# zichunhao/lgn-autoencoder

Hardware: AMD Instinct MI355X
Metric: jets/sec fwd+bwd, 30-particle maxdim=2 bs=512 (higher is better)
Workload: dtype f64

## Files before the change

### include/lgn_amd.h

```cpp
#ifndef LGN_AMD_H
#define LGN_AMD_H

#include <stddef.h>
#include <stdint.h>

#ifdef __cplusplus
extern "C" {
#endif

#define LGN_AMD_ABI_VERSION 19

int lgn_abi_version(void);
const char* lgn_last_error(void);

int lgn_level_fwd_f64(int B, int N, int C, int CO, int decoder,
                      const double* s_in, const double* v_in, const double* p, const uint8_t* mask,
                      const double* ra, const double* rb, const double* rc,
                      const double* w0, const double* b0, const double* w1, const double* b1,
                      const double* wm0, const double* wm1,
                      double* ag0, double* ag1, double* s_out, double* v_out, void* stream);

int lgn_level_bwd_partial_rows(int B, int N, int decoder, int* rows_mix, int* rows_rad);
int lgn_level_rad_partial_len(int C, int decoder);
int lgn_level_jet_split(int B, int N);
// ... 96 lines not shown
  double jet_loss_scale;
} lgn_net_desc;
#define LGN_REAL_SUM 0
#define LGN_REAL_REAL 1
#define LGN_REAL_IMAG 2
#define LGN_REAL_MEAN 3
#define LGN_REAL_NORM 4
#define LGN_LOSS_CHAMFER 0
#define LGN_LOSS_MSE 1
#define LGN_LOSS_HUNGARIAN 2
#define LGN_LOSS_EMD 3
typedef struct lgn_loss_desc {
  int kind;
  int abs_coord;
  int polar_coord;
  double scale;
} lgn_loss_desc;
#define LGN_POOL_MIN 0
#define LGN_POOL_MAX 1
#define LGN_POOL_MEAN 2
#define LGN_POOL_MIX 3
#define LGN_POOL(n, avg, o0, o1, o2, o3) ((n) | ((avg) << 3) | ((o0) << 4) | ((o1) << 6) | ((o2) << 8) | ((o3) << 10))
#define LGN_NET_NO_STATIC 1
#define LGN_NET_DEC_PAIRWISE 2
#define LGN_NET_LEVEL_V2 4
#define LGN_NET_MLP_V1 8
#define LGN_NET_MOMENTS_V1 16
#define LGN_NET_BWD_ORDERED 64
#define LGN_NET_DEC_UNFUSED 256
#define LGN_NET_MOMENTS_SPLIT 512
#define LGN_NET_MLP_BWD1 1024
#define LGN_NET_MLP_FULLTILE 2048
#define LGN_NET_LIVE_SCALARS 4096
#define LGN_NET_SPLIT_TAIL 128

#define LGN_LDS_LIMIT (160 * 1024)
long long lgn_encoder_end_lds_bytes(int N, int C0, int K, int CL, int Ts, int Tv, int pool);
long long lgn_decoder_end_lds_bytes(int N, int C0, int Tin, int CL);
long long lgn_junction_lds_bytes(int N, int CL, int Ts, int Tv, int pool, int C0);

int lgn_step_param_slots(const lgn_net_desc* d, int decoder);
long long lgn_step_workspace_doubles(const lgn_net_desc* d);
int lgn_step_fwd_bwd_f64(const lgn_net_desc* d, const double* params, double* grads, long long n_params,
                         const int64_t* enc_off, const int64_t* dec_off, const double* p4, const double* target,
                         const uint8_t* mask, const double* in_scalars, double* workspace, long long workspace_doubles,
                         double* recon, double* loss_part, const lgn_loss_desc* loss, int* assignment ,
                         int* status , void* stream);
#define LGN_FINALIZE_SCRATCH 2048
int lgn_step_finalize_f64(double* params, double* grads, long long n_params, const double* loss_part, int n_loss,
                          double l1_lambda, double* adam_m, double* adam_v, long long* step_dev,
                          double lr, double beta1, double beta2, double eps, int do_adam, double* loss_out, void* stream);
int lgn_step_train_f64(const lgn_net_desc* d, double* params, double* grads, long long n_params, const int64_t* enc_off,
                       const int64_t* dec_off, const double* p4, const double* target, const uint8_t* mask, const double* in_scalars,
                       double* workspace, long long workspace_doubles, double* recon, double* loss_part, int n_loss, double l1_lambda,
                       double* adam_m, double* adam_v, long long* step_dev, double lr, double beta1, double beta2, double eps,
                       int do_adam, double* loss_out, const lgn_loss_desc* loss, int* assignment ,
                       int* status , void* stream);

#define LGN_OPT_ADAM 0
#define LGN_OPT_RMSPROP 1
typedef struct {
  int kind;
  double l1_lambda, l2_lambda, lr, eps;
  double beta1, beta2;
  double alpha, momentum;
} lgn_optim_desc;
// ... 223 lines not shown
```

### lgn-autoencoder_amd/csrc/mlp_chain.hip

```cpp
#include "lds.hpp"
#include "ops.hpp"

namespace lgn {

namespace { LGN_STAMP_DECL }
#ifdef LGN_STAMPS
#define DSTAMP(i) do { if (threadIdx.x == 256 && blockIdx.x == 0) g_stamps[i] = clock64(); } while (0)
#else
#define DSTAMP(i) do { } while (0)
#endif
LGN_STAMP_READER(lgn_debug_stamps_mlp_chain)

namespace chain {

__host__ __device__ constexpr int stride2mod4(int x) { return x + ((6 - (x & 3)) & 3); }

__device__ __forceinline__ void lds_barrier() {
  __builtin_amdgcn_sched_barrier(0);
  __builtin_amdgcn_fence(__ATOMIC_RELEASE, "workgroup", "local");
  __builtin_amdgcn_s_barrier();
  __builtin_amdgcn_fence(__ATOMIC_ACQUIRE, "workgroup", "local");
  __builtin_amdgcn_sched_barrier(0);
}
template <int N, int P, class LoadF, class MmaF, class SideF>
// ... 223 lines not shown
  mfma_stream<N, LOOKAHEAD>(
      [&](int i) {
        const int u = It::tile(i), ks = It::ks(i);
        return u < NF ? wa[4 * ks * S + 16 * u] : wt[4 * ks * S + 4 * (u - NF)];
      },
      [&](int i, double av) {
        const int u = It::tile(i), ks = It::ks(i);
        if (u < NF) gin[u] = __builtin_amdgcn_mfma_f64_16x16x4f64(av, gpre[ks >> 2][ks & 3], gin[u], 0, 0, 0);
        else gin[NTO - 1][u - NF] = mfma4(av, gpre[ks >> 2][ks & 3], gin[NTO - 1][u - NF]);
      },
      [&](int i) {
        const int u = It::tile(i), ks = It::ks(i);
        constexpr int k1 = KS > 6 ? 5 : KS > 1 ? 1 : 0, k2 = KS > 6 ? 6 : KS > 2 ? 2 : k1, k3 = k2 + 1 < KS ? k2 + 1 : k2;
#pragma unroll
        for (int r = 0; r < 4; ++r)
          if (u > 0 && u < NF && ks == (r < 2 ? k1 : k2)) fin(u > 0 ? u - 1 : 0, r);
#pragma unroll
        for (int q = 0; q < NB; ++q)
          if (TH && u == 1 && NF > 1 && ks == k3) fin(NTO - 1, q);
        ext(i);
      });
}
template <class G, int NTO, bool TH_, class FinF>
__device__ __forceinline__ void fin_last(FinF fin, int r) {
  constexpr bool TH = TH_ && NTO == G::NT;
  if (!TH) fin(NTO - 1, r);
  else {
    fin(NTO - 2, r);
    if (NTO == 2 && r < G::NB) fin(NTO - 1, r);
  }
}

template <class G>
__device__ __forceinline__ double* saved_ptr(const MlpArgs<double>& a, int wave, int lane) {
  return a.h_saved + ((size_t)blockIdx.x * 4 + wave) * (G::NH * G::NT * 256) + lane * 4;
}
template <class G>
constexpr int saved_pieces() { return 2 * G::NT; }
template <class G, int NTI>
__device__ __forceinline__ void save_piece(double* hs, int l, const v4d (&h)[NTI], int j) {
  const v2d v = {h[j >> 1][2 * (j & 1)], h[j >> 1][2 * (j & 1) + 1]};
  __builtin_nontemporal_store(v, reinterpret_cast<v2d*>(hs + (l * G::NT + (j >> 1)) * 256 + 2 * (j & 1)));
}
template <class G>
__device__ __forceinline__ void load_piece(const double* hs, int l, v4d (&h)[G::NT], int j) {
  const v2d v = __builtin_nontemporal_load(reinterpret_cast<const v2d*>(hs + (l * G::NT + (j >> 1)) * 256 + 2 * (j & 1)));
  h[j >> 1][2 * (j & 1)] = v[0];
  h[j >> 1][2 * (j & 1) + 1] = v[1];
}

template <class G>
__device__ __forceinline__ void load_x(const MlpArgs<double>& a, int row, int g, v4d (&xb)[1]) {
  const bool rok = row < a.M;
#pragma unroll
  for (int r = 0; r < 4; ++r) {
    const int f = 4 * r + g;
    const bool ok = r < G::KS0 && rok && f < G::D;
    const double x = a.s_in[ok ? (size_t)(f & 1) * a.M * a.C + (size_t)row * a.C + (f >> 1) : 0];
    xb[0][r] = ok ? x : 0.0;
  }
}

template <int H, int D, bool GEN, bool SAVE, bool TWO = false, bool TH = false>
__global__ __launch_bounds__(TWO ? 512 : 256) void mlp_chain_fwd_kernel(MlpArgs<double> a) {
  using G = Geo<H, D>;
  const int tid = threadIdx.x, lane = tid & 63, wave = __builtin_amdgcn_readfirstlane(tid >> 6);
  const int c = lane & 15, g = lane >> 4;
  const int row = blockIdx.x * 64 + wave * 16 + c;
  extern __shared__ __align__(16) unsigned char smem_raw[];
  double* Wl = reinterpret_cast<double*>(smem_raw);
  WRegs<G> wrA, wrB;
  STAMP(0);
  STAMP_LIFE_BEGIN();
  if constexpr (TWO) {
    if (wave >= 4) {
      const int st = tid - 256;
      stage_prologue<G, false>(a, Wl, wrA, wrB, st);
      lds_barrier();
#define LGN_STAGE_STEP(Q)                                                                                            \
  _Pragma("unroll") for (int j = 0; j < stage_pieces<G>(); ++j) stage_piece<G, false, Q>(a, Wl, wrA, wrB, st, j);    \
  lds_barrier();
      LGN_STAGE_STEP(0) LGN_STAGE_STEP(1) LGN_STAGE_STEP(2) LGN_STAGE_STEP(3) LGN_STAGE_STEP(4) LGN_STAGE_STEP(5)
#undef LGN_STAGE_STEP
      return;
    }
  }
  v4d xb[1];
  load_x<G>(a, row, g, xb);
  if constexpr (!TWO) stage_prologue<G, false>(a, Wl, wrA, wrB, tid);
  lds_barrier();
  STAMP(1);
  v4d h0[G::NT], h1[G::NT];
  double* hs = SAVE ? saved_ptr<G>(a, wave, lane) : nullptr;
#define LGN_CHAIN_STEP(Q, HIN, HOUT, KS, NTI)                                                                        \
  layer_fwd<G, KS, NTI, GEN, TH, (Q == 3)>(Wl + (Q & 1) * G::WSIZE, HIN, HOUT, c, g, a.act, [&](int i) {           \
    constexpr int NI = Items<G, KS, TH>::N;                                                                          \
    if (!TWO && !LGN_DBG_NOSTAGE) deal<NI, stage_pieces<G>()>(i, [&](int j) { stage_piece<G, false, Q>(a, Wl, wrA, wrB, tid, j); });      \
    if (SAVE && Q > 0) deal<NI, 2 * NTI>(i, [&](int j) { save_piece<G>(hs, Q - 1, HIN, j); });                      \
  });                                                                                                                \
  lds_barrier();                                                                                                     \
  STAMP(2 + Q);
  LGN_CHAIN_STEP(0, xb, h0, G::KS0, 1)
  LGN_CHAIN_STEP(1, h0, h1, G::KSH, G::NT)
  LGN_CHAIN_STEP(2, h1, h0, G::KSH, G::NT)
  LGN_CHAIN_STEP(3, h0, h1, G::KSH, G::NT)
  LGN_CHAIN_STEP(4, h1, h0, G::KSH, G::NT)
  LGN_CHAIN_STEP(5, h0, h1, G::KSH, G::NT)
#undef LGN_CHAIN_STEP
  if (SAVE) {
#pragma unroll
    for (int j = 0; j < saved_pieces<G>(); ++j) save_piece<G>(hs, G::NH - 1, h1, j);
  }
  const v4d y = layer_out<G>(Wl + (G::NH & 1) * G::WSIZE, h1, c, g);
#pragma unroll
  for (int r = 0; r < 4; ++r) {
    const int o = 4 * r + g;
    if (o < D && row < a.M) a.s_out[mlp_out_index(a, o & 1, row, o >> 1)] = y[r];
  }
  STAMP(8);
  STAMP_LIFE_END();
}

template <class G, int NTI>
__device__ __forceinline__ void publish_piece(double* T, const v4d (&v)[NTI], int wave, int c, int g, int j) {
  T[(4 * j + g) * G::SR + 16 * wave + c] = v[j >> 2][j & 3];
}
template <class G, int L, int NU, class SideF>
__device__ __forceinline__ void dw_unit(const double* Gt, const double* Xt, double* part, int t, int u0, int c, int g, SideF side) {
  constexpr int SR = G::SR, HO = G::hout(L), HI = G::hin(L), N = 16 * NU, P = 6;
  const double* ga = Gt + (16 * t + c) * SR + g;
  const double* xb = Xt + (16 * u0 + c) * SR + g;
  double* pW = part + G::off_w(L);
  v4d acc[NU];
#pragma unroll
  for (int u = 0; u < NU; ++u) acc[u] = v4d{0, 0, 0, 0};
  double dbs = 0.0, qa[16], qx[N];
  auto load = [&](int i) {
    qx[i] = xb[16 * (i >> 4) * SR + 4 * (i & 15)];
    if (i < 16) qa[i] = ga[4 * i];
  };
  auto store = [&](int u, int r) {
    const int o = 16 * t + 4 * r + g, k = 16 * (u0 + u) + c;
    if (o < HO && k < HI) __builtin_nontemporal_store(acc[u][r], &pW[o * HI + k]);
  };
// ... 29 lines not shown
    if (wave < G::NT) { dw_unit<G, L, 1>(Gt, Xt, part, wave, 0, c, g, side); return true; }
  } else {
    const int t = (wave + L) & 3;
    if (t < G::NT) { dw_unit<G, L, G::NT>(Gt, Xt, part, t, 0, c, g, side); return true; }
  }
  return false;
}

template <int H, int D, bool GEN, bool SAVE, bool TH = false>
__global__ __launch_bounds__(256) void mlp_chain_bwd_kernel(MlpArgs<double> a) {
  using G = Geo<H, D>;
  constexpr int NT = G::NT, NH = G::NH;
  const int tid = threadIdx.x, lane = tid & 63, wave = __builtin_amdgcn_readfirstlane(tid >> 6);
  const int c = lane & 15, g = lane >> 4;
  const int row = blockIdx.x * 64 + wave * 16 + c;
  extern __shared__ __align__(16) unsigned char smem_raw[];
  double* Wl = reinterpret_cast<double*>(smem_raw);
  double* Gt = Wl + 2 * G::WSIZE;
  double* Xt = Gt + 2 * G::TSIZE;
  double* part = a.part + (size_t)blockIdx.x * a.psize;
  WRegs<G> wrA, wrB;
  STAMP(10);
  v4d xb[1];
  load_x<G>(a, row, g, xb);
  v4d gout[1];
#pragma unroll
  for (int r = 0; r < 4; ++r) {
    const int o = 4 * r + g;
    const bool ok = o < D && row < a.M;
    const double x = a.g_out[ok ? mlp_out_index(a, o & 1, row, o >> 1) : 0];
    gout[0][r] = ok ? x : 0.0;
  }
  v4d h[NH][NT];
  const double* hs = SAVE ? saved_ptr<G>(a, wave, lane) : nullptr;
  if constexpr (SAVE) {
    issue_image<G, NH>(a, wrA, tid);
    issue_image<G, NH - 1>(a, wrB, tid);
#pragma unroll
    for (int j = 0; j < saved_pieces<G>(); ++j) load_piece<G>(hs, NH - 1, h[NH - 1], j);
#pragma unroll
    for (int j = 0; j < saved_pieces<G>(); ++j) load_piece<G>(hs, NH - 2, h[NH - 2], j);
    commit_image<G, NH>(Wl, wrA, tid);
    issue_image<G, NH - 2>(a, wrA, tid);
    lds_barrier();
    STAMP(11);
  } else {
    stage_prologue<G, true>(a, Wl, wrA, wrB, tid);
    lds_barrier();
    STAMP(11);
#define LGN_CHAIN_STEP(Q, HIN, KS, NTI)                                                                              \
  layer_fwd<G, KS, NTI, GEN, TH>(Wl + (Q & 1) * G::WSIZE, HIN, h[Q], c, g, a.act, [&](int i) {                      \
    deal<Items<G, KS, TH>::N, stage_pieces<G>()>(i, [&](int j) { stage_piece<G, true, Q>(a, Wl, wrA, wrB, tid, j); });  \
  });                                                                                                                \
  lds_barrier();                                                                                                     \
  STAMP(12 + Q);
    LGN_CHAIN_STEP(0, xb, G::KS0, 1)
    LGN_CHAIN_STEP(1, h[0], G::KSH, NT)
    LGN_CHAIN_STEP(2, h[1], G::KSH, NT)
    LGN_CHAIN_STEP(3, h[2], G::KSH, NT)
    LGN_CHAIN_STEP(4, h[3], G::KSH, NT)
    LGN_CHAIN_STEP(5, h[4], G::KSH, NT)
#undef LGN_CHAIN_STEP
  }
  v4d gpA[NT] = {}, gpB[NT] = {}, gin[NT];
  {
    constexpr int NI = Items<G, G::KS0, TH>::N, NSV = SAVE && NH >= 3 ? saved_pieces<G>() : 0, NPC = 4 + 4 * NT + stage_pieces<G>() + NSV;
    auto fin = [&](int u, int r) {
      double y = gin[u][r] * act_slope_t<GEN>(h[NH - 1][u][r], a.act);
      pin(y);
      gpA[u][r] = y;
    };
    layer_bwd<G, G::KS0, NT, 1, TH>(Wl + 0 * G::WSIZE, gout, gin, c, g, fin, [&](int i) {
      deal<NI, NPC>(i, [&](int j) {
        if (j < 4) publish_piece<G, 1>(Gt, gout, wave, c, g, j);
        else if (j < 4 + 4 * NT) publish_piece<G, NT>(Xt, h[NH - 1], wave, c, g, j - 4);
        else if (j < 4 + 4 * NT + stage_pieces<G>()) stage_piece<G, true, NH>(a, Wl, wrA, wrB, tid, j - 4 - 4 * NT);
        else if constexpr (NSV > 0) load_piece<G>(hs, NH - 3, h[NH >= 3 ? NH - 3 : 0], j - 4 - 4 * NT - stage_pieces<G>());
      });
    });
#pragma unroll
    for (int r = 0; r < 4; ++r) fin_last<G, NT, TH>(fin, r);
    lds_barrier();
    STAMP(18);
  }
#define LGN_CHAIN_BSTEP(L, GP, GN)                                                                                   \
  {                                                                                                                  \
    constexpr int q_ = 2 * NH - (L), NI = Items<G, G::KSH, TH>::N, NSV = SAVE && (L) >= 3 ? saved_pieces<G>() : 0,               \
                  NPC = 8 * NT + stage_pieces<G>() + NSV;                                                            \
    auto fin = [&](int u, int r) {                                                                                   \
      double y = gin[u][r] * act_slope_t<GEN>(h[(L) - 1][u][r], a.act);                                              \
      pin(y);                                                                                                        \
      GN[u][r] = y;                                                                                                  \
    };                                                                                                               \
    layer_bwd<G, G::KSH, NT, NT, TH>(Wl + (q_ & 1) * G::WSIZE, GP, gin, c, g, fin, [&](int i) {                          \
      deal<NI, NPC>(i, [&](int j) {                                                                                  \
        if (j < 4 * NT) publish_piece<G, NT>(Gt + ((L) & 1) * G::TSIZE, GP, wave, c, g, j);                          \
        else if (j < 8 * NT) publish_piece<G, NT>(Xt + ((L) & 1) * G::TSIZE, h[(L) - 1], wave, c, g, j - 4 * NT);    \
        else if (j < 8 * NT + stage_pieces<G>()) stage_piece<G, true, q_>(a, Wl, wrA, wrB, tid, j - 8 * NT);         \
        else if constexpr (NSV > 0) load_piece<G>(hs, (L) - 3, h[(L) >= 3 ? (L) - 3 : 0], j - 8 * NT - stage_pieces<G>()); \
      });                                                                                                            \
    });                                                                                                              \
    auto tail = [&](int i) {                                                                                         \
      if (i == 1) { fin_last<G, NT, TH>(fin, 0); fin_last<G, NT, TH>(fin, 1); }                                                                \
      if (i == 2) { fin_last<G, NT, TH>(fin, 2); fin_last<G, NT, TH>(fin, 3); }                                                                \
    };                                                                                                               \
    if (!dw_layer<G, (L) + 1>(Gt + (((L) + 1) & 1) * G::TSIZE, Xt + (((L) + 1) & 1) * G::TSIZE, part, wave, c, g, tail)) {   \
      tail(1);                                                                                                       \
      tail(2);                                                                                                       \
    }                                                                                                                \
    lds_barrier();                                                                                                   \
    STAMP(12 + q_);                                                                                                  \
  }
  LGN_CHAIN_BSTEP(5, gpA, gpB)
  LGN_CHAIN_BSTEP(4, gpB, gpA)
  LGN_CHAIN_BSTEP(3, gpA, gpB)
  LGN_CHAIN_BSTEP(2, gpB, gpA)
  LGN_CHAIN_BSTEP(1, gpA, gpB)
#undef LGN_CHAIN_BSTEP
  {
    v4d gx[1];
    layer_bwd<G, G::KSH, 1, NT, TH>(Wl + 0 * G::WSIZE, gpB, gx, c, g, [&](int, int) {}, [&](int i) {
      deal<G::KSH, 4 * NT + 4>(i, [&](int j) {
        if (j < 4 * NT) publish_piece<G, NT>(Gt, gpB, wave, c, g, j);
        else publish_piece<G, 1>(Xt, xb, wave, c, g, j - 4 * NT);
      });
    });
    auto tail = [&](int i) {
      if (i >= 1 && i <= 4) {
        const int f = 4 * (i - 1) + g;
        if (f < D && row < a.M) a.g_in[mlp_out_index(a, f & 1, row, f >> 1)] = gx[0][i - 1];
      }
    };
// ... 91 lines not shown
#pragma unroll
  for (int i = 0; i < P; ++i) load(i);
  __builtin_amdgcn_sched_barrier(0);
#pragma unroll
  for (int i = 0; i < N; ++i) {
    if (i + P < N) load(i + P);
    if (i < 16) acc = __builtin_amdgcn_mfma_f64_16x16x4f64(qa[i], qx[i], acc, 0, 0, 0);
    else strip = mfma4(qa[i], qx[i], strip);
    if (i >= 17 && i <= 20) __builtin_nontemporal_store(acc[i - 17], &pW[(16 * t + 4 * (i - 17) + g) * H + 16 * u + c]);
    side(i);
    __builtin_amdgcn_sched_barrier(0);
  }
  __builtin_nontemporal_store(strip, tr ? &pW[(16 * u + c) * H + 32 + g] : &pW[(32 + g) * H + 16 * u + c]);
  if (w == 3) {
    const double* ca = Gt + (32 + (c & 3)) * SR + 16 * (c >> 2) + g;
    const double* cb = Xt + (32 + (c & 3)) * SR + 16 * (c >> 2) + g;
    double v = 0.0;
#pragma unroll
    for (int sk = 0; sk < 4; ++sk) v = mfma4(ca[4 * sk], cb[4 * sk], v);
    v += shfl_xor(v, 4);
    v += shfl_xor(v, 8);
    if (c < 4) __builtin_nontemporal_store(v, &pW[(32 + g) * H + 32 + c]);
  } else {
    double d4[4] = {0.0, 0.0, 0.0, 0.0};
#pragma unroll
    for (int sk = 0; sk < 16; ++sk) d4[sk & 3] += w == 1 ? qa[16 + sk] : qa[sk];
    double dbs = (d4[0] + d4[1]) + (d4[2] + d4[3]);
    dbs += shfl_xor(dbs, 16);
    dbs += shfl_xor(dbs, 32);
    if (g == 0 && (w != 1 || c < 4)) __builtin_nontemporal_store(dbs, &part[G::off_b(L) + (w == 1 ? 32 : 16 * t) + c]);
  }
}

template <int H, int D, bool GEN, bool TH = false>
__global__ __launch_bounds__(512) void mlp_chain_bwd2_kernel(MlpArgs<double> a) {
  using G = Geo<H, D>;
  constexpr int NT = G::NT, NH = G::NH;
  const int lane = threadIdx.x & 63, wave = __builtin_amdgcn_readfirstlane((int)threadIdx.x >> 6);
  const int w4 = wave & 3;
  const int c = lane & 15, g = lane >> 4;
  extern __shared__ __align__(16) unsigned char smem_raw[];
  double* Wl = reinterpret_cast<double*>(smem_raw);
  double* Gt = Wl + 2 * G::WSIZE;
  double* Xt = Gt + 2 * G::TSIZE;
  STAMP(10);
  if (wave >= 4) {
    __builtin_amdgcn_s_setprio(2);
    const int tid = (int)threadIdx.x - 256;
    double* part = a.part + (size_t)blockIdx.x * a.psize;
    WRegs<G> wrA, wrB;
    stage_prologue<G, true>(a, Wl, wrA, wrB, tid);
    lds_barrier();
#define LGN_STAGE_ALL(Q)                                                                                             \
  _Pragma("unroll") for (int j = 0; j < stage_pieces<G>(); ++j) stage_piece<G, true, Q>(a, Wl, wrA, wrB, tid, j);
#define LGN_STAGE_STEP(Q) LGN_STAGE_ALL(Q) lds_barrier();
    LGN_STAGE_STEP(0) LGN_STAGE_STEP(1) LGN_STAGE_STEP(2) LGN_STAGE_STEP(3) LGN_STAGE_STEP(4) LGN_STAGE_STEP(5)
    LGN_STAGE_STEP(6)
    constexpr bool THIN3 = TH && NT == 3 && G::R == 4, EVEN = NT == 3 && !THIN3;
    double* qs = Xt + 2 * G::TSIZE;
#define LGN_DW_STEP(L)                                                                                               \
  {                                                                                                                  \
    constexpr int q_ = 2 * NH - (L), NS = stage_pieces<G>(), L1 = (L) + 1;                                           \
    constexpr bool HID = EVEN && L1 >= 1 && L1 < NH, HID3 = THIN3 && L1 >= 1 && L1 < NH;                             \
    constexpr int NI = HID ? 36 : HID3 ? 32 : (L1 == NH || L1 == 0) ? 16 : 16 * NT;                                  \
    auto side = [&](int i) { deal<NI, NS>(i, [&](int j) { stage_piece<G, true, q_>(a, Wl, wrA, wrB, tid, j); }); };  \
    if constexpr (EVEN && L1 + 1 >= 1 && L1 + 1 < NH) {                                                              \
      if (w4 == 1) dw_quarter_sum<G, (L1 + 1 < NH ? L1 + 1 : 1)>(qs + ((L1 + 1) & 1) * 1024, part, lane, c, g);     \
    }                                                                                                                \
    if constexpr (HID3) {                                                                                            \
      dw_thin3<G, (HID3 ? L1 : 1)>(Gt + (L1 & 1) * G::TSIZE, Xt + (L1 & 1) * G::TSIZE, part, w4, c, g, side);        \
    } else if constexpr (HID) {                                                                                      \
      dw_hidden3<G, (HID ? L1 : 1)>(Gt + (L1 & 1) * G::TSIZE, Xt + (L1 & 1) * G::TSIZE, part, qs + (L1 & 1) * 1024, w4, lane, c, g, side); \
    } else if (!dw_layer<G, L1>(Gt + (L1 & 1) * G::TSIZE, Xt + (L1 & 1) * G::TSIZE, part, w4, c, g, side)) {         \
      LGN_STAGE_ALL(q_)                                                                                              \
    }                                                                                                                \
    DSTAMP(44 + (L));                                                                                                \
    lds_barrier();                                                                                                   \
  }
    LGN_DW_STEP(5) LGN_DW_STEP(4) LGN_DW_STEP(3) LGN_DW_STEP(2) LGN_DW_STEP(1) LGN_DW_STEP(0)
#undef LGN_DW_STEP
#undef LGN_STAGE_STEP
#undef LGN_STAGE_ALL
    if constexpr (EVEN && NH >= 2) {
      if (w4 == 1) dw_quarter_sum<G, 1>(qs + 1024, part, lane, c, g);
    }
    dw_layer<G, 0>(Gt, Xt, part, w4, c, g, [&](int) {});
    return;
  }
  const int row = blockIdx.x * 64 + wave * 16 + c;
  v4d xb[1];
  load_x<G>(a, row, g, xb);
  v4d gout[1];
#pragma unroll
  for (int r = 0; r < 4; ++r) {
    const int o = 4 * r + g;
    const bool ok = o < D && row < a.M;
    const double x = a.g_out[ok ? mlp_out_index(a, o & 1, row, o >> 1) : 0];
    gout[0][r] = ok ? x : 0.0;
  }
  v4d h[NH][NT];
  lds_barrier();
  STAMP(11);
#define LGN_CHAIN_STEP(Q, HIN, KS, NTI)                                                                              \
  layer_fwd<G, KS, NTI, GEN, TH>(Wl + (Q & 1) * G::WSIZE, HIN, h[Q], c, g, a.act, [&](int) {});                          \
  lds_barrier();                                                                                                     \
  STAMP(12 + Q);
  LGN_CHAIN_STEP(0, xb, G::KS0, 1)
  LGN_CHAIN_STEP(1, h[0], G::KSH, NT)
  LGN_CHAIN_STEP(2, h[1], G::KSH, NT)
  LGN_CHAIN_STEP(3, h[2], G::KSH, NT)
  LGN_CHAIN_STEP(4, h[3], G::KSH, NT)
  LGN_CHAIN_STEP(5, h[4], G::KSH, NT)
#undef LGN_CHAIN_STEP
  v4d gpA[NT] = {}, gpB[NT] = {}, gin[NT];
  {
    constexpr int NI = Items<G, G::KS0, TH>::N, NPC = 4 + 4 * NT;
    auto fin = [&](int u, int r) {
      double y = gin[u][r] * act_slope_t<GEN>(h[NH - 1][u][r], a.act);
      pin(y);
      gpA[u][r] = y;
    };
    layer_bwd<G, G::KS0, NT, 1, TH>(Wl + 0 * G::WSIZE, gout, gin, c, g, fin, [&](int i) {
      deal<NI, NPC>(i, [&](int j) {
        if (j < 4) publish_piece<G, 1>(Gt, gout, wave, c, g, j);
        else publish_piece<G, NT>(Xt, h[NH - 1], wave, c, g, j - 4);
      });
    });
#pragma unroll
    for (int r = 0; r < 4; ++r) fin_last<G, NT, TH>(fin, r);
    lds_barrier();
    STAMP(18);
  }
#define LGN_CHAIN_BSTEP(L, GP, GN)                                                                                   \
  {                                                                                                                  \
    constexpr int q_ = 2 * NH - (L), NI = Items<G, G::KSH, TH>::N, NPC = 8 * NT;                                                 \
    auto fin = [&](int u, int r) {                                                                                   \
      double y = gin[u][r] * act_slope_t<GEN>(h[(L) - 1][u][r], a.act);                                              \
      pin(y);                                                                                                        \
      GN[u][r] = y;                                                                                                  \
    };                                                                                                               \
    layer_bwd<G, G::KSH, NT, NT, TH>(Wl + (q_ & 1) * G::WSIZE, GP, gin, c, g, fin, [&](int i) {                          \
      deal<NI, NPC>(i, [&](int j) {                                                                                  \
        if (j < 4 * NT) publish_piece<G, NT>(Gt + ((L) & 1) * G::TSIZE, GP, wave, c, g, j);                          \
        else publish_piece<G, NT>(Xt + ((L) & 1) * G::TSIZE, h[(L) - 1], wave, c, g, j - 4 * NT);                    \
      });                                                                                                            \
    });                                                                                                              \
    STAMP(56 + (L));                                                                                                 \
    _Pragma("unroll") for (int r = 0; r < 4; ++r) fin_last<G, NT, TH>(fin, r);                                                    \
    STAMP(50 + (L));                                                                                                 \
    lds_barrier();                                                                                                   \
    STAMP(12 + q_);                                                                                                  \
  }
  LGN_CHAIN_BSTEP(5, gpA, gpB)
  LGN_CHAIN_BSTEP(4, gpB, gpA)
  LGN_CHAIN_BSTEP(3, gpA, gpB)
  LGN_CHAIN_BSTEP(2, gpB, gpA)
  LGN_CHAIN_BSTEP(1, gpA, gpB)
#undef LGN_CHAIN_BSTEP
  {
    v4d gx[1];
    layer_bwd<G, G::KSH, 1, NT, TH>(Wl + 0 * G::WSIZE, gpB, gx, c, g, [&](int, int) {}, [&](int i) {
      deal<G::KSH, 4 * NT + 4>(i, [&](int j) {
        if (j < 4 * NT) publish_piece<G, NT>(Gt, gpB, wave, c, g, j);
        else publish_piece<G, 1>(Xt, xb, wave, c, g, j - 4 * NT);
      });
    });
#pragma unroll
    for (int r = 0; r < 4; ++r) {
      const int f = 4 * r + g;
      if (f < D && row < a.M) a.g_in[mlp_out_index(a, f & 1, row, f >> 1)] = gx[0][r];
    }
    lds_barrier();
    STAMP(25);
  }
}

template <class G>
__device__ __forceinline__ double* saved_ptr16(const MlpArgs<double>& a, int lane) {
  return a.h_saved + (size_t)blockIdx.x * (G::NH * G::NT * 256) + lane * 4;
}
// ... 515 lines not shown
  using G = Geo<H, D, 128>;
  const int nblk = cdiv(a.M, 16);
  const size_t smem = backward ? G::bwd_bytes() : G::fwd_bytes();
  if (backward) LGN_CHECK_ARG(a.psize == G::psize(), "cgmlp: psize %d, expected %d", a.psize, G::psize());
  LGN_CHECK_ARG(!a.h_saved || a.h_rows >= nblk * 16, "cgmlp: the saved-activation buffer has %d rows per layer, %d rows need %d",
                a.h_rows, a.M, nblk * 16);
  void (*kern)(MlpArgs<double>);
  if (backward) kern = a.h_saved ? (a.act == 0 ? mlp_chain_bwd16_kernel<H, D, false, true> : mlp_chain_bwd16_kernel<H, D, true, true>)
                                 : (a.act == 0 ? mlp_chain_bwd16_kernel<H, D, false, false> : mlp_chain_bwd16_kernel<H, D, true, false>);
  else kern = a.h_saved ? (a.act == 0 ? mlp_chain_fwd16_kernel<H, D, false, true> : mlp_chain_fwd16_kernel<H, D, true, true>)
                        : (a.act == 0 ? mlp_chain_fwd16_kernel<H, D, false, false> : mlp_chain_fwd16_kernel<H, D, true, false>);
  return lds_launch(kern, "cgmlp (16-row)", dim3(nblk), dim3(backward ? 256 : 192), smem, stream, a);
}

template <int H, int D, bool TH>
static int launch_fwd(const MlpArgs<double>& a, hipStream_t stream) {
  using G = Geo<H, D>;
  static_assert(G::fwd_bytes() <= LGN_LDS_LIMIT, "LDS budget");
  const bool two = !(a.flags & LVL_MLP_BWD1);
  auto kern = two ? (a.act == 0 ? mlp_chain_fwd_kernel<H, D, false, false, true, TH> : mlp_chain_fwd_kernel<H, D, true, false, true, TH>)
                  : (a.act == 0 ? mlp_chain_fwd_kernel<H, D, false, false, false, TH> : mlp_chain_fwd_kernel<H, D, true, false, false, TH>);
  return lds_launch(kern, "cgmlp forward (wide)", dim3(cdiv(a.M, 64)), dim3(two ? 512 : 256), G::fwd_bytes(), stream, a);
}

template <int H, int D, bool TH>
static int launch(const MlpArgs<double>& a, bool backward, hipStream_t stream) {
  using G = Geo<H, D>;
  const int nblk = cdiv(a.M, 64);
  const size_t smem = backward ? G::bwd_bytes() : G::fwd_bytes();
  static_assert(G::bwd_bytes() <= LGN_LDS_LIMIT, "LDS budget");
  if (backward) LGN_CHECK_ARG(a.psize == G::psize(), "cgmlp: psize %d, expected %d", a.psize, G::psize());
  LGN_CHECK_ARG(!a.h_saved || a.h_rows >= nblk * 64, "cgmlp: the saved-activation buffer has %d rows per layer, %d rows need %d",
                a.h_rows, a.M, nblk * 64);
  if (backward && !a.h_saved && !(a.flags & LVL_MLP_BWD1)) {
    auto k2 = a.act == 0 ? mlp_chain_bwd2_kernel<H, D, false, TH> : mlp_chain_bwd2_kernel<H, D, true, TH>;
    const size_t smem2 = smem - (TH && G::NT == 3 && G::R == 4 ? sizeof(double) * 2 * 1024 : 0);
    return lds_launch(k2, "cgmlp backward (two roles)", dim3(nblk), dim3(512), smem2, stream, a);
  }
  if (!backward && !a.h_saved && !(a.flags & LVL_MLP_BWD1)) {
    auto k2 = a.act == 0 ? mlp_chain_fwd_kernel<H, D, false, false, true, TH> : mlp_chain_fwd_kernel<H, D, true, false, true, TH>;
    return lds_launch(k2, "cgmlp forward (two roles)", dim3(nblk), dim3(512), smem, stream, a);
  }
  auto kern = a.h_saved ? (a.act == 0 ? (backward ? mlp_chain_bwd_kernel<H, D, false, true, TH> : mlp_chain_fwd_kernel<H, D, false, true, false, TH>)
                                      : (backward ? mlp_chain_bwd_kernel<H, D, true, true, TH> : mlp_chain_fwd_kernel<H, D, true, true, false, TH>))
                        : (a.act == 0 ? (backward ? mlp_chain_bwd_kernel<H, D, false, false, TH> : mlp_chain_fwd_kernel<H, D, false, false, false, TH>)
                                      : (backward ? mlp_chain_bwd_kernel<H, D, true, false, TH> : mlp_chain_fwd_kernel<H, D, true, false, false, TH>));
  return lds_launch(kern, "cgmlp", dim3(nblk), dim3(256), smem, stream, a);
}
template <int H, int D>
static int launch_thin(const MlpArgs<double>& a, bool backward, hipStream_t stream) {
  static_assert(Geo<H, D>::THIN, "a last tile of at most eight neurons");
  return (a.flags & LVL_MLP_FULLTILE) ? launch<H, D, false>(a, backward, stream) : launch<H, D, true>(a, backward, stream);
}

}

int mlp_chain_dispatch(const MlpArgs<double>& a, bool backward, hipStream_t stream) {
  if ((a.flags & LVL_MLP_V1) || a.nlin != 7) return -2;
  if (mlp_rows_per_workgroup(a.M, a.H) != 64) {
    if (!(a.flags & LVL_MLP_BWD1) && (!backward || a.h_saved)) {
      if (a.H == 48 && a.C == 4) return chain::launch16s<48, 8>(a, backward, stream);
      if (a.H == 36 && a.C == 3) return chain::launch16s<36, 6>(a, backward, stream);
    }
    if (a.H == 48 && a.C == 4) return chain::launch16<48, 8>(a, backward, stream);
    if (a.H == 36 && a.C == 3) return chain::launch16<36, 6>(a, backward, stream);
    if (a.H == 24 && a.C == 2) return chain::launch16<24, 4>(a, backward, stream);
    if (a.H == 12 && a.C == 1) return chain::launch16<12, 2>(a, backward, stream);
    return -2;
  }
  if (a.H == 48 && a.C == 4) return chain::launch<48, 8, false>(a, backward, stream);
  if (a.H == 36 && a.C == 3) return chain::launch_thin<36, 6>(a, backward, stream);
  if (a.H == 24 && a.C == 2) return chain::launch_thin<24, 4>(a, backward, stream);
  if (a.H == 12 && a.C == 1) return chain::launch<12, 2, false>(a, backward, stream);
// ... 11 lines not shown
```

### lgn-autoencoder_amd/csrc/step.hip

```cpp
#include <stdlib.h>

#include <algorithm>
#include <vector>

#include "net.hpp"
#include "../../include/lgn_amd.h"

namespace lgn {
namespace {

inline size_t r16(size_t n) { return (n + 15) & ~size_t(15); }

struct Bump {
  double* base;
  size_t off = 0;
  double* here() const { return base ? base + off : nullptr; }
  double* take(size_t n) {
    double* p = here();
    off += r16(n);
    return p;
  }
};

struct Deferred {
// ... 228 lines not shown
}

bool stage_keeps_chamfer(const StageLoss* al) { return !al || (al->kind == LGN_LOSS_EMD && al->emd.chamfer_weight > 0.0); }
double chamfer_scale(const StageLoss* al) { return al ? al->emd.chamfer_weight : 1.0; }

int stage_loss_train(const StageLoss& L, int B, int N, int C, const double* v, const double* wo1, const double* target, int method,
                     double* recon, double* loss_part, double* g_v, double* part, hipStream_t st) {
  if (L.kind == LGN_LOSS_EMD) return dec_output_emd_loss(B, N, C, v, wo1, target, method, L.emd, recon, loss_part, g_v, part, st);
  return dec_output_assign_loss(B, N, C, v, wo1, target, method, L.al, recon, loss_part, g_v, part, st);
}
int stage_loss_eval(const StageLoss& L, int B, int N, int C, const double* v, const double* wo1, const double* target, int method,
                    double* recon_real, double* loss_part, hipStream_t st) {
  if (L.kind == LGN_LOSS_EMD) return dec_output_emd_eval(B, N, C, v, wo1, target, method, L.emd, recon_real, loss_part, st);
  return dec_output_assign_eval(B, N, C, v, wo1, target, method, L.al, recon_real, loss_part, st);
}

struct NetBuf {
  double *s[5], *v[5], *smix[4], *ag0[4], *ag1[4];
  double* hsave[4];
  double* sep[4];
};
void carve_net(Bump& b, const lgn_net_desc& d, bool dec, size_t BN, bool last_mlp_bwd, NetBuf& n) {
  const int* ch = dec ? d.dec_channels : d.enc_channels;
  const int L = d.n_levels;
  for (int l = 0; l <= L; ++l) {
    n.s[l] = b.take(2 * BN * ch[l]);
    n.v[l] = b.take(8 * BN * ch[l]);
  }
  for (int l = 0; l < L; ++l) {
    n.smix[l] = b.take(2 * BN * ch[l + 1]);
    n.ag0[l] = b.take(4 * BN * ch[l]);
    n.ag1[l] = b.take(16 * BN * ch[l]);
    n.sep[l] = dec ? b.take((size_t)d.B * sep_sums_doubles(ch[l])) : nullptr;
    const size_t hs = (last_mlp_bwd || l + 1 < L) && BN <= mlp_save_max_rows()
                          ? mlp_saved_doubles((int)BN, d.mlp_hidden_mul * 2 * ch[l + 1], d.mlp_nlin) : 0;
    n.hsave[l] = hs ? b.take(hs) : nullptr;
  }
}

struct BwdScratch {
  double *gs[2], *gv[2];
  double *gsmix, *g_ag;
  double *zeros_s, *g_p, *g_lat_s, *tail_cnt;
  size_t zero_doubles;
  double* zero0() const { return tail_cnt < zeros_s ? tail_cnt : zeros_s; }
  double* tot[4];
  double* parts;
  size_t parts_size;
};
void carve_level_grads(Bump& b, size_t BN, int cmax, BwdScratch& k) {
  for (int q = 0; q < 2; ++q) {
    k.gs[q] = b.take(2 * BN * cmax);
    k.gv[q] = b.take(8 * BN * cmax);
  }
  k.gsmix = b.take(2 * BN * cmax);
  k.g_ag = b.take(20 * BN * cmax);
}
inline size_t tot_doubles(int C, bool dec) { return rad_partial_size(C, dec) + 16; }

size_t net_parts(const lgn_net_desc& d, bool dec, int N) {
  const int* ch = dec ? d.dec_channels : d.enc_channels;
  int rm, rr;
  level_bwd_partial_rows(d.B, N, dec, d.flags, &rm, &rr);
  size_t sum = 0;
  for (int l = 0; l < d.n_levels; ++l) {
    const int H = d.mlp_hidden_mul * 2 * ch[l + 1];
    sum += r16((size_t)rm * 4 * ch[l + 1] * 5 * ch[l]) + r16((size_t)rr * rad_partial_size(ch[l], dec)) +
// ... 1153 lines not shown
```

### lgn-autoencoder_amd/lgn/_native.py

```python
from __future__ import annotations

import ctypes as C
import os
from typing import Optional, Sequence

import torch

_HERE = os.path.dirname(os.path.abspath(__file__))
LIB_PATH = os.environ.get("LGN_AMD_LIB") or os.path.join(_HERE, "_lib", "liblgn_amd.so")
ABI_VERSION = 19
FINALIZE_SCRATCH = 2048
FINALIZE_OPT_SCRATCH = 4096

_lib: Optional[C.CDLL] = None

_vp, _i, _ip = C.c_void_p, C.c_int, C.POINTER(C.c_int)

_SIGNATURES = {
    "lgn_level_fwd_f64": [_i] * 5 + [_vp] * 18,
    "lgn_level_bwd_partial_rows": [_i, _i, _i, _ip, _ip],
    "lgn_level_rad_partial_len": [_i, _i],
    "lgn_level_jet_split": [_i, _i],
    "lgn_cg_product_fwd_f64": [_i] * 8 + [_vp] * 7,
    "lgn_cg_product_bwd_f64": [_i] * 8 + [_vp] * 9,
# ... 54 lines not shown
            need = max(need, L.lgn_junction_lds_bytes(n, ch[-1], ts, tv, code, decoder.num_channels[0]))
    if decoder is not None:
        ch = decoder.num_channels
        need = max(need, L.lgn_decoder_end_lds_bytes(decoder.num_output_particles, ch[0], decoder.tau_latent_vectors, ch[-1]))
    return 0 <= need <= LDS_LIMIT


def pool_blocks(code: int) -> int:
    if code == 0:
        return 2
    return 1 if (code >> 3) & 1 else code & 7


class NetDesc(C.Structure):
    _fields_ = [("B", C.c_int), ("N", C.c_int), ("n_levels", C.c_int), ("enc_channels", C.c_int * 5),
                ("dec_channels", C.c_int * 5), ("tau_s", C.c_int), ("tau_v", C.c_int), ("mlp_hidden_mul", C.c_int),
                ("mlp_nlin", C.c_int), ("tau_v_in", C.c_int),
                ("enc_tables", _tp * 4), ("dec_tables", _tp * 4),
                ("enc_Q", C.c_int * 5), ("enc_qs", C.c_int * 5), ("enc_qv", C.c_int * 5),
                ("dec_Q", C.c_int * 5), ("dec_qs", C.c_int * 5), ("dec_qv", C.c_int * 5), ("flags", C.c_int),
                ("activation", C.c_int), ("n_in_scalars", C.c_int), ("latent_pool", C.c_int), ("dec_N", C.c_int),
                ("get_real", C.c_int), ("jet_loss_scale", C.c_double)]

    def __init__(self, *a, **kw):
        super().__init__(*a, **kw)
        self.flags = net_flags()


NET_NO_STATIC = 1
_NET_FLAG_ENV = {"LGN_AMD_NO_STATIC": 1, "LGN_AMD_DEC_PAIRWISE": 2, "LGN_AMD_LEVEL_V2": 4, "LGN_AMD_MLP_V1": 8,
                 "LGN_AMD_MOMENTS_V1": 16, "LGN_AMD_BWD_ORDERED": 64, "LGN_AMD_LIVE_SCALARS": 4096, "LGN_AMD_SPLIT_TAIL": 128, "LGN_AMD_DEC_UNFUSED": 256, "LGN_AMD_MOMENTS_SPLIT": 512,
                 "LGN_AMD_MLP_BWD1": 1024, "LGN_AMD_MLP_FULLTILE": 2048,
                 "LGN_AMD_DEC_STORE_AG": 16384}
ACTIVATIONS = {"leakyrelu": 0, "relu": 1, "elu": 2, "sigmoid": 3, "logsigmoid": 4, "atan": 5}


def activation_id(name: str) -> int:
    try:
        return ACTIVATIONS[name.lower()]
    except KeyError:
        raise ValueError(f"Activation function {name} not implemented!") from None


def net_flags() -> int:
    return sum(bit for name, bit in _NET_FLAG_ENV.items() if os.environ.get(name, "") == "1")


class LossDesc(C.Structure):
    _fields_ = [("kind", C.c_int), ("abs_coord", C.c_int), ("polar_coord", C.c_int), ("scale", C.c_double)]


class OptimDesc(C.Structure):
    _fields_ = [("kind", C.c_int), ("l1_lambda", C.c_double), ("l2_lambda", C.c_double), ("lr", C.c_double), ("eps", C.c_double),
                ("beta1", C.c_double), ("beta2", C.c_double), ("alpha", C.c_double), ("momentum", C.c_double)]


class EmdOpts(C.Structure):
    _fields_ = [("R", C.c_double), ("beta", C.c_double), ("norm", C.c_int), ("periodic_phi", C.c_int)]


class SinkhornOpts(C.Structure):
    _fields_ = [("base", EmdOpts), ("epsilon", C.c_double), ("tol", C.c_double), ("max_iter", C.c_int), ("debias", C.c_int)]


class EMDLossDesc(C.Structure):
    _fields_ = [("base", LossDesc), ("opts", EmdOpts), ("chamfer_weight", C.c_double)]


def loss_ref(desc):
    if desc is None:
        return None
    return C.byref(desc.base) if isinstance(desc, EMDLossDesc) else C.byref(desc)


OPT_ADAM, OPT_RMSPROP = 0, 1
LOSS_CHAMFER, LOSS_MSE, LOSS_HUNGARIAN, LOSS_EMD = 0, 1, 2, 3
ASSIGN_NMAX = 192
_dp = C.POINTER(NetDesc)
# ... 377 lines not shown
```

Before: 1.132 million.

## Save MLP hidden activations in two-role kernels instead of recomputing in backward

Adds a default-on keep flag that allocates the saved-activation buffer even for large row counts. The two-role forward and backward MLP chain kernels get a SAVE variant: the forward writes each hidden layer to global memory, and the backward loads those layers in place of recomputing the forward chain. The save layout changes to contiguous per-lane lines, and thin tiles skip storing their padding registers. The trade is extra global memory traffic and workspace in exchange for removing the forward recompute inside backward.

```diff
diff --git a/include/lgn_amd.h b/include/lgn_amd.h
--- a/include/lgn_amd.h
+++ b/include/lgn_amd.h
@@ -152,6 +152,7 @@
 #define LGN_NET_MLP_BWD1 1024
 #define LGN_NET_MLP_FULLTILE 2048
 #define LGN_NET_LIVE_SCALARS 4096
+#define LGN_NET_MLP_KEEP 8192
 #define LGN_NET_SPLIT_TAIL 128
 
 #define LGN_LDS_LIMIT (160 * 1024)
diff --git a/lgn-autoencoder_amd/csrc/mlp_chain.hip b/lgn-autoencoder_amd/csrc/mlp_chain.hip
--- a/lgn-autoencoder_amd/csrc/mlp_chain.hip
+++ b/lgn-autoencoder_amd/csrc/mlp_chain.hip
@@ -279,11 +279,27 @@
 }
 
 template <class G>
-__device__ __forceinline__ double* saved_ptr(const MlpArgs<double>& a, int wave, int lane) {
-  return a.h_saved + ((size_t)blockIdx.x * 4 + wave) * (G::NH * G::NT * 256) + lane * 4;
+__device__ __forceinline__ double* line_ptr(const MlpArgs<double>& a, int wave, int lane) {
+  return a.h_saved + ((size_t)blockIdx.x * 4 + wave) * (G::NH * G::NT * 256) + lane * 2;
+}
+template <class G, int NTI>
+__device__ __forceinline__ void save_line(double* hs, int l, const v4d (&h)[NTI], int j) {
+  const v2d v = {h[j >> 1][2 * (j & 1)], h[j >> 1][2 * (j & 1) + 1]};
+  __builtin_nontemporal_store(v, reinterpret_cast<v2d*>(hs + (l * 2 * G::NT + j) * 128));
+}
+template <class G>
+__device__ __forceinline__ void load_line(const double* hs, int l, v4d (&h)[G::NT], int j) {
+  const v2d v = __builtin_nontemporal_load(reinterpret_cast<const v2d*>(hs + (l * 2 * G::NT + j) * 128));
+  h[j >> 1][2 * (j & 1)] = v[0];
+  h[j >> 1][2 * (j & 1) + 1] = v[1];
 }
 template <class G>
 constexpr int saved_pieces() { return 2 * G::NT; }
+template <class G, bool TH>
+constexpr int line_pieces() {
+  static_assert(!TH || (G::THIN && G::NB <= 2), "a thin tile's registers 2 and 3 are padding");
+  return 2 * G::NT - (TH ? 1 : 0);
+}
 template <class G, int NTI>
 __device__ __forceinline__ void save_piece(double* hs, int l, const v4d (&h)[NTI], int j) {
   const v2d v = {h[j >> 1][2 * (j & 1)], h[j >> 1][2 * (j & 1) + 1]};
@@ -338,12 +354,12 @@
   lds_barrier();
   STAMP(1);
   v4d h0[G::NT], h1[G::NT];
-  double* hs = SAVE ? saved_ptr<G>(a, wave, lane) : nullptr;
+  double* hs = SAVE ? line_ptr<G>(a, wave, lane) : nullptr;
 #define LGN_CHAIN_STEP(Q, HIN, HOUT, KS, NTI)                                                                        \
   layer_fwd<G, KS, NTI, GEN, TH, (Q == 3)>(Wl + (Q & 1) * G::WSIZE, HIN, HOUT, c, g, a.act, [&](int i) {           \
     constexpr int NI = Items<G, KS, TH>::N;                                                                          \
     if (!TWO && !LGN_DBG_NOSTAGE) deal<NI, stage_pieces<G>()>(i, [&](int j) { stage_piece<G, false, Q>(a, Wl, wrA, wrB, tid, j); });      \
-    if (SAVE && Q > 0) deal<NI, 2 * NTI>(i, [&](int j) { save_piece<G>(hs, Q - 1, HIN, j); });                      \
+    if (SAVE && Q > 0) deal<NI, (Q > 0 ? line_pieces<G, TH>() : 1)>(i, [&](int j) { save_line<G>(hs, Q - 1, HIN, j); });            \
   });                                                                                                                \
   lds_barrier();                                                                                                     \
   STAMP(2 + Q);
@@ -356,7 +372,7 @@
 #undef LGN_CHAIN_STEP
   if (SAVE) {
 #pragma unroll
-    for (int j = 0; j < saved_pieces<G>(); ++j) save_piece<G>(hs, G::NH - 1, h1, j);
+    for (int j = 0; j < line_pieces<G, TH>(); ++j) save_line<G>(hs, G::NH - 1, h1, j);
   }
   const v4d y = layer_out<G>(Wl + (G::NH & 1) * G::WSIZE, h1, c, g);
 #pragma unroll
@@ -452,14 +468,18 @@
     gout[0][r] = ok ? x : 0.0;
   }
   v4d h[NH][NT];
-  const double* hs = SAVE ? saved_ptr<G>(a, wave, lane) : nullptr;
+  if constexpr (SAVE && TH) {
+#pragma unroll
+    for (int l = 0; l < NH; ++l) h[l][NT - 1] = v4d{0, 0, 0, 0};
+  }
+  const double* hs = SAVE ? line_ptr<G>(a, wave, lane) : nullptr;
   if constexpr (SAVE) {
     issue_image<G, NH>(a, wrA, tid);
     issue_image<G, NH - 1>(a, wrB, tid);
 #pragma unroll
-    for (int j = 0; j < saved_pieces<G>(); ++j) load_piece<G>(hs, NH - 1, h[NH - 1], j);
-#pragma unroll
-    for (int j = 0; j < saved_pieces<G>(); ++j) load_piece<G>(hs, NH - 2, h[NH - 2], j);
+    for (int j = 0; j < line_pieces<G, TH>(); ++j) load_line<G>(hs, NH - 1, h[NH - 1], j);
+#pragma unroll
+    for (int j = 0; j < line_pieces<G, TH>(); ++j) load_line<G>(hs, NH - 2, h[NH - 2], j);
     commit_image<G, NH>(Wl, wrA, tid);
     issue_image<G, NH - 2>(a, wrA, tid);
     lds_barrier();
@@ -484,7 +504,7 @@
   }
   v4d gpA[NT] = {}, gpB[NT] = {}, gin[NT];
   {
-    constexpr int NI = Items<G, G::KS0, TH>::N, NSV = SAVE && NH >= 3 ? saved_pieces<G>() : 0, NPC = 4 + 4 * NT + stage_pieces<G>() + NSV;
+    constexpr int NI = Items<G, G::KS0, TH>::N, NSV = SAVE && NH >= 3 ? line_pieces<G, TH>() : 0, NPC = 4 + 4 * NT + stage_pieces<G>() + NSV;
     auto fin = [&](int u, int r) {
       double y = gin[u][r] * act_slope_t<GEN>(h[NH - 1][u][r], a.act);
       pin(y);
@@ -495,7 +515,7 @@
         if (j < 4) publish_piece<G, 1>(Gt, gout, wave, c, g, j);
         else if (j < 4 + 4 * NT) publish_piece<G, NT>(Xt, h[NH - 1], wave, c, g, j - 4);
         else if (j < 4 + 4 * NT + stage_pieces<G>()) stage_piece<G, true, NH>(a, Wl, wrA, wrB, tid, j - 4 - 4 * NT);
-        else if constexpr (NSV > 0) load_piece<G>(hs, NH - 3, h[NH >= 3 ? NH - 3 : 0], j - 4 - 4 * NT - stage_pieces<G>());
+        else if constexpr (NSV > 0) load_line<G>(hs, NH - 3, h[NH >= 3 ? NH - 3 : 0], j - 4 - 4 * NT - stage_pieces<G>());
       });
     });
 #pragma unroll
@@ -505,7 +525,7 @@
   }
 #define LGN_CHAIN_BSTEP(L, GP, GN)                                                                                   \
   {                                                                                                                  \
-    constexpr int q_ = 2 * NH - (L), NI = Items<G, G::KSH, TH>::N, NSV = SAVE && (L) >= 3 ? saved_pieces<G>() : 0,               \
+    constexpr int q_ = 2 * NH - (L), NI = Items<G, G::KSH, TH>::N, NSV = SAVE && (L) >= 3 ? line_pieces<G, TH>() : 0,          \
                   NPC = 8 * NT + stage_pieces<G>() + NSV;                                                            \
     auto fin = [&](int u, int r) {                                                                                   \
       double y = gin[u][r] * act_slope_t<GEN>(h[(L) - 1][u][r], a.act);                                              \
@@ -517,7 +537,7 @@
         if (j < 4 * NT) publish_piece<G, NT>(Gt + ((L) & 1) * G::TSIZE, GP, wave, c, g, j);                          \
         else if (j < 8 * NT) publish_piece<G, NT>(Xt + ((L) & 1) * G::TSIZE, h[(L) - 1], wave, c, g, j - 4 * NT);    \
         else if (j < 8 * NT + stage_pieces<G>()) stage_piece<G, true, q_>(a, Wl, wrA, wrB, tid, j - 8 * NT);         \
-        else if constexpr (NSV > 0) load_piece<G>(hs, (L) - 3, h[(L) >= 3 ? (L) - 3 : 0], j - 8 * NT - stage_pieces<G>()); \
+        else if constexpr (NSV > 0) load_line<G>(hs, (L) - 3, h[(L) >= 3 ? (L) - 3 : 0], j - 8 * NT - stage_pieces<G>()); \
       });                                                                                                            \
     });                                                                                                              \
     auto tail = [&](int i) {                                                                                         \
@@ -675,7 +695,7 @@
   }
 }
 
-template <int H, int D, bool GEN, bool TH = false>
+template <int H, int D, bool GEN, bool TH = false, bool SAVE = false>
 __global__ __launch_bounds__(512) void mlp_chain_bwd2_kernel(MlpArgs<double> a) {
   using G = Geo<H, D>;
   constexpr int NT = G::NT, NH = G::NH;
@@ -692,12 +712,20 @@
     const int tid = (int)threadIdx.x - 256;
     double* part = a.part + (size_t)blockIdx.x * a.psize;
     WRegs<G> wrA, wrB;
-    stage_prologue<G, true>(a, Wl, wrA, wrB, tid);
-    lds_barrier();
 #define LGN_STAGE_ALL(Q)                                                                                             \
   _Pragma("unroll") for (int j = 0; j < stage_pieces<G>(); ++j) stage_piece<G, true, Q>(a, Wl, wrA, wrB, tid, j);
 #define LGN_STAGE_STEP(Q) LGN_STAGE_ALL(Q) lds_barrier();
-    LGN_STAGE_STEP(0) LGN_STAGE_STEP(1) LGN_STAGE_STEP(2) LGN_STAGE_STEP(3) LGN_STAGE_STEP(4) LGN_STAGE_STEP(5)
+    if constexpr (SAVE) {
+      issue_image<G, NH>(a, wrA, tid);
+      issue_image<G, NH - 1>(a, wrB, tid);
+      commit_image<G, NH>(Wl, wrA, tid);
+      issue_image<G, NH - 2>(a, wrA, tid);
+      lds_barrier();
+    } else {
+      stage_prologue<G, true>(a, Wl, wrA, wrB, tid);
+      lds_barrier();
+      LGN_STAGE_STEP(0) LGN_STAGE_STEP(1) LGN_STAGE_STEP(2) LGN_STAGE_STEP(3) LGN_STAGE_STEP(4) LGN_STAGE_STEP(5)
+    }
     LGN_STAGE_STEP(6)
     constexpr bool THIN3 = TH && NT == 3 && G::R == 4, EVEN = NT == 3 && !THIN3;
     double* qs = Xt + 2 * G::TSIZE;
@@ -742,22 +770,36 @@
     gout[0][r] = ok ? x : 0.0;
   }
   v4d h[NH][NT];
-  lds_barrier();
-  STAMP(11);
+  if constexpr (SAVE && TH) {
+#pragma unroll
+    for (int l = 0; l < NH; ++l) h[l][NT - 1] = v4d{0, 0, 0, 0};
+  }
+  const double* hs = SAVE ? line_ptr<G>(a, wave, lane) : nullptr;
+  if constexpr (SAVE) {
+#pragma unroll
+    for (int j = 0; j < line_pieces<G, TH>(); ++j) load_line<G>(hs, NH - 1, h[NH - 1], j);
+#pragma unroll
+    for (int j = 0; j < line_pieces<G, TH>(); ++j) load_line<G>(hs, NH - 2, h[NH - 2], j);
+    lds_barrier();
+    STAMP(11);
+  } else {
+    lds_barrier();
+    STAMP(11);
 #define LGN_CHAIN_STEP(Q, HIN, KS, NTI)                                                                              \
   layer_fwd<G, KS, NTI, GEN, TH>(Wl + (Q & 1) * G::WSIZE, HIN, h[Q], c, g, a.act, [&](int) {});                          \
   lds_barrier();                                                                                                     \
   STAMP(12 + Q);
-  LGN_CHAIN_STEP(0, xb, G::KS0, 1)
-  LGN_CHAIN_STEP(1, h[0], G::KSH, NT)
-  LGN_CHAIN_STEP(2, h[1], G::KSH, NT)
-  LGN_CHAIN_STEP(3, h[2], G::KSH, NT)
-  LGN_CHAIN_STEP(4, h[3], G::KSH, NT)
-  LGN_CHAIN_STEP(5, h[4], G::KSH, NT)
+    LGN_CHAIN_STEP(0, xb, G::KS0, 1)
+    LGN_CHAIN_STEP(1, h[0], G::KSH, NT)
+    LGN_CHAIN_STEP(2, h[1], G::KSH, NT)
+    LGN_CHAIN_STEP(3, h[2], G::KSH, NT)
+    LGN_CHAIN_STEP(4, h[3], G::KSH, NT)
+    LGN_CHAIN_STEP(5, h[4], G::KSH, NT)
 #undef LGN_CHAIN_STEP
+  }
   v4d gpA[NT] = {}, gpB[NT] = {}, gin[NT];
   {
-    constexpr int NI = Items<G, G::KS0, TH>::N, NPC = 4 + 4 * NT;
+    constexpr int NI = Items<G, G::KS0, TH>::N, NSV = SAVE && NH >= 3 ? line_pieces<G, TH>() : 0, NPC = 4 + 4 * NT + NSV;
     auto fin = [&](int u, int r) {
       double y = gin[u][r] * act_slope_t<GEN>(h[NH - 1][u][r], a.act);
       pin(y);
@@ -766,7 +808,8 @@
     layer_bwd<G, G::KS0, NT, 1, TH>(Wl + 0 * G::WSIZE, gout, gin, c, g, fin, [&](int i) {
       deal<NI, NPC>(i, [&](int j) {
         if (j < 4) publish_piece<G, 1>(Gt, gout, wave, c, g, j);
-        else publish_piece<G, NT>(Xt, h[NH - 1], wave, c, g, j - 4);
+        else if (j < 4 + 4 * NT) publish_piece<G, NT>(Xt, h[NH - 1], wave, c, g, j - 4);
+        else if constexpr (NSV > 0) load_line<G>(hs, NH - 3, h[NH >= 3 ? NH - 3 : 0], j - 4 - 4 * NT);
       });
     });
 #pragma unroll
@@ -776,7 +819,8 @@
   }
 #define LGN_CHAIN_BSTEP(L, GP, GN)                                                                                   \
   {                                                                                                                  \
-    constexpr int q_ = 2 * NH - (L), NI = Items<G, G::KSH, TH>::N, NPC = 8 * NT;                                                 \
+    constexpr int q_ = 2 * NH - (L), NI = Items<G, G::KSH, TH>::N, NSV = SAVE && (L) >= 3 ? line_pieces<G, TH>() : 0, \
+                  NPC = 8 * NT + NSV;                                                                                \
     auto fin = [&](int u, int r) {                                                                                   \
       double y = gin[u][r] * act_slope_t<GEN>(h[(L) - 1][u][r], a.act);                                              \
       pin(y);                                                                                                        \
@@ -785,10 +829,11 @@
     layer_bwd<G, G::KSH, NT, NT, TH>(Wl + (q_ & 1) * G::WSIZE, GP, gin, c, g, fin, [&](int i) {                          \
       deal<NI, NPC>(i, [&](int j) {                                                                                  \
         if (j < 4 * NT) publish_piece<G, NT>(Gt + ((L) & 1) * G::TSIZE, GP, wave, c, g, j);                          \
-        else publish_piece<G, NT>(Xt + ((L) & 1) * G::TSIZE, h[(L) - 1], wave, c, g, j - 4 * NT);                    \
+        else if (j < 8 * NT) publish_piece<G, NT>(Xt + ((L) & 1) * G::TSIZE, h[(L) - 1], wave, c, g, j - 4 * NT);    \
+        else if constexpr (NSV > 0) load_line<G>(hs, (L) - 3, h[(L) >= 3 ? (L) - 3 : 0], j - 8 * NT);                \
       });                                                                                                            \
     });                                                                                                              \
-    STAMP(56 + (L));                                                                                                 \
+    STAMP(56 + (L));                                                                                               \
     _Pragma("unroll") for (int r = 0; r < 4; ++r) fin_last<G, NT, TH>(fin, r);                                                    \
     STAMP(50 + (L));                                                                                                 \
     lds_barrier();                                                                                                   \
@@ -1370,13 +1415,15 @@
   if (backward) LGN_CHECK_ARG(a.psize == G::psize(), "cgmlp: psize %d, expected %d", a.psize, G::psize());
   LGN_CHECK_ARG(!a.h_saved || a.h_rows >= nblk * 64, "cgmlp: the saved-activation buffer has %d rows per layer, %d rows need %d",
                 a.h_rows, a.M, nblk * 64);
-  if (backward && !a.h_saved && !(a.flags & LVL_MLP_BWD1)) {
-    auto k2 = a.act == 0 ? mlp_chain_bwd2_kernel<H, D, false, TH> : mlp_chain_bwd2_kernel<H, D, true, TH>;
+  if (backward && !(a.flags & LVL_MLP_BWD1)) {
+    auto k2 = a.h_saved ? (a.act == 0 ? mlp_chain_bwd2_kernel<H, D, false, TH, true> : mlp_chain_bwd2_kernel<H, D, true, TH, true>)
+                        : (a.act == 0 ? mlp_chain_bwd2_kernel<H, D, false, TH, false> : mlp_chain_bwd2_kernel<H, D, true, TH, false>);
     const size_t smem2 = smem - (TH && G::NT == 3 && G::R == 4 ? sizeof(double) * 2 * 1024 : 0);
     return lds_launch(k2, "cgmlp backward (two roles)", dim3(nblk), dim3(512), smem2, stream, a);
   }
-  if (!backward && !a.h_saved && !(a.flags & LVL_MLP_BWD1)) {
-    auto k2 = a.act == 0 ? mlp_chain_fwd_kernel<H, D, false, false, true, TH> : mlp_chain_fwd_kernel<H, D, true, false, true, TH>;
+  if (!backward && !(a.flags & LVL_MLP_BWD1)) {
+    auto k2 = a.h_saved ? (a.act == 0 ? mlp_chain_fwd_kernel<H, D, false, true, true, TH> : mlp_chain_fwd_kernel<H, D, true, true, true, TH>)
+                        : (a.act == 0 ? mlp_chain_fwd_kernel<H, D, false, false, true, TH> : mlp_chain_fwd_kernel<H, D, true, false, true, TH>);
     return lds_launch(k2, "cgmlp forward (two roles)", dim3(nblk), dim3(512), smem, stream, a);
   }
   auto kern = a.h_saved ? (a.act == 0 ? (backward ? mlp_chain_bwd_kernel<H, D, false, true, TH> : mlp_chain_fwd_kernel<H, D, false, true, false, TH>)
diff --git a/lgn-autoencoder_amd/csrc/step.hip b/lgn-autoencoder_amd/csrc/step.hip
--- a/lgn-autoencoder_amd/csrc/step.hip
+++ b/lgn-autoencoder_amd/csrc/step.hip
@@ -284,7 +284,7 @@
     n.ag0[l] = b.take(4 * BN * ch[l]);
     n.ag1[l] = b.take(16 * BN * ch[l]);
     n.sep[l] = dec ? b.take((size_t)d.B * sep_sums_doubles(ch[l])) : nullptr;
-    const size_t hs = (last_mlp_bwd || l + 1 < L) && BN <= mlp_save_max_rows()
+    const size_t hs = (last_mlp_bwd || l + 1 < L) && (BN <= mlp_save_max_rows() || (d.flags & LGN_NET_MLP_KEEP))
                           ? mlp_saved_doubles((int)BN, d.mlp_hidden_mul * 2 * ch[l + 1], d.mlp_nlin) : 0;
     n.hsave[l] = hs ? b.take(hs) : nullptr;
   }
diff --git a/lgn-autoencoder_amd/lgn/_native.py b/lgn-autoencoder_amd/lgn/_native.py
--- a/lgn-autoencoder_amd/lgn/_native.py
+++ b/lgn-autoencoder_amd/lgn/_native.py
@@ -110,6 +110,7 @@
                  "LGN_AMD_MOMENTS_V1": 16, "LGN_AMD_BWD_ORDERED": 64, "LGN_AMD_LIVE_SCALARS": 4096, "LGN_AMD_SPLIT_TAIL": 128, "LGN_AMD_DEC_UNFUSED": 256, "LGN_AMD_MOMENTS_SPLIT": 512,
                  "LGN_AMD_MLP_BWD1": 1024, "LGN_AMD_MLP_FULLTILE": 2048,
                  "LGN_AMD_DEC_STORE_AG": 16384}
+NET_MLP_KEEP = 8192
 ACTIVATIONS = {"leakyrelu": 0, "relu": 1, "elu": 2, "sigmoid": 3, "logsigmoid": 4, "atan": 5}
 
 
@@ -121,7 +122,8 @@
 
 
 def net_flags() -> int:
-    return sum(bit for name, bit in _NET_FLAG_ENV.items() if os.environ.get(name, "") == "1")
+    keep = 0 if os.environ.get("LGN_AMD_MLP_RECOMPUTE", "") == "1" else NET_MLP_KEEP
+    return keep + sum(bit for name, bit in _NET_FLAG_ENV.items() if os.environ.get(name, "") == "1")
 
 
 class LossDesc(C.Structure):
```

New measurement: 1.153 million, median of 6. 1.02x the previous value.
